# COMPiLELab/krylov_robustness

Measured on NVIDIA B200. Metric: krylov_matvecs_per_sec, higher is better.
Workload: dtype f64

## Files before the change

### krylov_robustness_b200/csrc/api.cu

```cuda
#include <memory>
#include <thread>
#include "common.cuh"
#include "csr.cuh"
#include "spmm.cuh"
#include "dense.cuh"
#include "slq.cuh"
#include "theta_table.h"
#include "smalldense.cuh"
#include "pairs.cuh"
#include "pairs_small.cuh"
#include "expmv.cuh"
#include "tsdense.cuh"
#include "smallgemm.cuh"
#include "vecops.cuh"
#include "blockkrylov.cuh"
#include "entries.cuh"
#include "entries_local.cuh"
#include "frechet.cuh"
#include "mctrace.cuh"
#include "nodepairs.cuh"

using namespace kr;

static void destroy_fun_update_result(kr_ctx* c);
// ... 295 lines not shown
        launch_spmm(ctx, A->dev, xb.p(), xb.panels, epi, nullptr, (int)k);
        download_cm(ctx, yb, Y, ldy);
    });
}

static void slq_finish(const SlqResult& R, int64_t m, double* tr, double* vals, double* alpha, double* beta) {
    if (tr) *tr = R.tr;
    const size_t k = R.vals.size();
    if (vals) std::memcpy(vals, R.vals.data(), k * sizeof(double));
    if (alpha || beta)
        for (int64_t j = 0; j < m; ++j)
            for (size_t c = 0; c < k; ++c) {
                if (alpha) alpha[c * m + j] = R.alpha[(size_t)j * k + c];
                if (beta) beta[c * m + j] = R.beta[(size_t)j * k + c];
            }
}

int kr_slq_trace_dev(kr_ctx* ctx, const kr_matrix* A, const kr_dense* Z, int64_t m, int fun, double* tr,
                     double* vals, double* alpha, double* beta) {
    return guarded([&] {
        if (!ctx || !A || !Z) fail(KR_ERR_ARG, "kr_slq_trace_dev: null argument");
        if (fun < 0 || fun > 2) fail(KR_ERR_ARG, "unsupported function selector");
        KR_CUDA(cudaSetDevice(ctx->device));
        PanelBuf W(ctx, Z->buf.n, Z->buf.cols);
        KR_CUDA(cudaMemcpyAsync(W.p(), Z->buf.p(), (size_t)W.elems() * sizeof(double), cudaMemcpyDeviceToDevice,
                                ctx->stream));
        SlqResult R = slq_run(ctx, A, W, (int)m, fun, alpha || beta);
        slq_finish(R, m, tr, vals, alpha, beta);
    });
}

}

template <class T>
static int slq_trace_host(kr_ctx* ctx, const kr_matrix* A, int64_t k, const T* Z, int64_t ldz, int64_t m, int fun,
                          double* tr, double* vals, double* alpha, double* beta) {
    return guarded([&] {
        if (!ctx || !A || !Z) fail(KR_ERR_ARG, "kr_slq_trace: null argument");
        if (fun < 0 || fun > 2) fail(KR_ERR_ARG, "unsupported function selector");
        KR_CUDA(cudaSetDevice(ctx->device));
        const int64_t n = A->dev.n;
        if (ldz < n) fail(KR_ERR_ARG, "The block vector b has wrong number of rows");
        if (k <= 0) fail(KR_ERR_ARG, "kr_slq_trace: no probe columns");
        std::vector<int64_t> cstart, cwidth;
        for (int64_t c0 = 0; c0 < k;) {
            const int64_t cw = std::min<int64_t>(k - c0, cstart.empty() ? 2 * PW : (cstart.size() == 1 ? 6 * PW : 8 * PW));
            cstart.push_back(c0);
            cwidth.push_back(cw);
            c0 += cw;
        }
        if (cstart.empty()) { cstart.push_back(0); cwidth.push_back(0); }
        const int64_t nch = (int64_t)cstart.size();
        if (!ctx->copy_stream) KR_CUDA(cudaStreamCreateWithFlags(&ctx->copy_stream, cudaStreamNonBlocking));
        std::vector<std::unique_ptr<PanelBuf>> W(nch);
        std::vector<std::unique_ptr<DevBuf<T>>> stage(nch);
        std::vector<cudaEvent_t> ready(nch, nullptr);
        for (int64_t c = 0; c < nch; ++c) {
            W[c].reset(new PanelBuf(ctx, n, (int)cwidth[c]));
            stage[c].reset(new DevBuf<T>(ctx, (size_t)std::max<int64_t>(n * cwidth[c], 1)));
        }
        KR_CUDA(cudaStreamSynchronize(ctx->stream));
        auto issue_copy = [&](int64_t c) {
            const int64_t c0 = cstart[c], cw = cwidth[c];
            if (n > 0 && cw > 0) {
                KR_CUDA(cudaMemcpy2DAsync(stage[c]->p, n * sizeof(T), Z + c0 * ldz, ldz * sizeof(T),
                                          n * sizeof(T), cw, cudaMemcpyHostToDevice, ctx->copy_stream));
                ctx->counters[3] += n * cw * (int64_t)sizeof(T);
            }
            cm_to_panel(ctx, stage[c]->p, n, *W[c], ctx->copy_stream);
            KR_CUDA(cudaEventCreateWithFlags(&ready[c], cudaEventDisableTiming));
            KR_CUDA(cudaEventRecord(ready[c], ctx->copy_stream));
        };
        std::vector<double> all_vals((size_t)k), all_a, all_b;
        if (alpha || beta) { all_a.resize((size_t)m * k); all_b.resize((size_t)m * k); }
        auto harvest = [&](int64_t c, SlqJob& job) {
            const int64_t c0 = cstart[c], cw = cwidth[c];
            SlqResult R = job.collect();
            for (int64_t q = 0; q < cw; ++q) all_vals[(size_t)(c0 + q)] = R.vals[(size_t)q];
            if (alpha || beta)
                for (int64_t j = 0; j < m; ++j)
                    for (int64_t q = 0; q < cw; ++q) {
                        all_a[(size_t)(j * k + c0 + q)] = R.alpha[(size_t)(j * cw + q)];
                        all_b[(size_t)(j * k + c0 + q)] = R.beta[(size_t)(j * cw + q)];
                    }
        };
        try {
            issue_copy(0);
            std::unique_ptr<SlqJob> prev;
            for (int64_t c = 0; c < nch; ++c) {
                KR_CUDA(cudaStreamWaitEvent(ctx->stream, ready[c], 0));
                std::unique_ptr<SlqJob> job(new SlqJob(ctx, A, *W[c], (int)m, fun, alpha || beta));
                job->mark();
                if (c + 1 < nch) issue_copy(c + 1);
                if (prev) harvest(c - 1, *prev);
                prev = std::move(job);
            }
            if (prev) harvest(nch - 1, *prev);
        } catch (...) {
            cudaStreamSynchronize(ctx->copy_stream);
            cudaStreamSynchronize(ctx->stream);
            for (auto e : ready) if (e) cudaEventDestroy(e);
            throw;
        }
        KR_CUDA(cudaStreamSynchronize(ctx->copy_stream));
        for (auto e : ready) if (e) cudaEventDestroy(e);
        SlqResult R;
        R.vals = all_vals;
        R.alpha = all_a;
        R.beta = all_b;
        double s = 0.0;
        for (int64_t q = 0; q < k; ++q) s += all_vals[(size_t)q];
        R.tr = k ? s / (double)k : 0.0;
        slq_finish(R, m, tr, vals, alpha, beta);
    });
// ... 53 lines not shown
```

### krylov_robustness_b200/csrc/csr.cuh

```cuda
#pragma once
#include <algorithm>
#include <map>
#include <numeric>

#include "common.cuh"

namespace kr {

struct RowTile {
    int start;
    int count;
    int lanes_log2;
    int pad;
};

struct CsrHost {
    int64_t n = 0;
    std::vector<int64_t> row_ptr;
    std::vector<int32_t> col;
    std::vector<double> val;
};

struct CsrDevView {
    int n;
// ... 12 lines not shown
    const double* __restrict__ dl_val;
    int dl_count;
};

#ifndef KR_SPMM_CAP
#define KR_SPMM_CAP 4096
#endif
#ifndef KR_SPMM_MAX_ROWS
#define KR_SPMM_MAX_ROWS 1024
#endif
constexpr int SPMM_CAP = KR_SPMM_CAP;
constexpr int SPMM_MAX_ROWS = KR_SPMM_MAX_ROWS;
constexpr int SPMM_LONG_ROW = 1024;
constexpr int64_t CSR_L2_RESIDENT_NNZ = 400000;

struct CsrDev {
    int64_t n = 0, nnz = 0;
    DevBuf<int> row_ptr, col, row_order, row_pos;
    DevBuf<double> val;
    DevBuf<RowTile> tiles;
    DevBuf<int> dl_tile_begin, dl_rowlocal, dl_pos, dl_col;
    DevBuf<double> dl_val;
    int dl_count = 0;
    std::vector<RowTile> tiles_host;
    std::vector<int> row_pos_host;
    int ntiles = 0;
    bool pattern_only = false;
    double uval = 1.0;
    CsrDevView view() const {
        CsrDevView v;
        v.n = (int)n;
        v.ntiles = ntiles;
        v.row_ptr = row_ptr.p;
        v.col = col.p;
        v.val = pattern_only ? nullptr : val.p;
        v.uval = uval;
        v.row_order = row_order.p;
        v.row_pos = row_pos.p;
        v.tiles = tiles.p;
        const bool dl = dl_count > 0;
        v.dl_tile_begin = dl ? dl_tile_begin.p : nullptr;
        v.dl_rowlocal = dl ? dl_rowlocal.p : nullptr;
        v.dl_pos = dl ? dl_pos.p : nullptr;
        v.dl_col = dl ? dl_col.p : nullptr;
        v.dl_val = dl ? dl_val.p : nullptr;
        v.dl_count = dl_count;
// ... 119 lines not shown
    D.nnz = nnz;
    D.pattern_only = P.uniform;
    D.uval = P.uval;
    D.row_ptr.reset(ctx, n + 1);
    D.row_ptr.upload(P.srp.data(), n + 1);
    D.col.reset(ctx, std::max<int64_t>(nnz, 1));
    if (nnz) D.col.upload(P.scol.data(), nnz);
    if (!P.uniform) {
        D.val.reset(ctx, std::max<int64_t>(nnz, 1));
        if (nnz) D.val.upload(P.sval.data(), nnz);
    } else {
        D.val.free();
    }
    D.ntiles = (int)P.tiles.size();
    D.row_order.reset(ctx, std::max<int64_t>(n, 1));
    if (n) D.row_order.upload(P.order.data(), n);
    std::vector<int> pos((size_t)std::max<int64_t>(n, 1), 0);
    for (int64_t s = 0; s < n; ++s) pos[(size_t)P.order[(size_t)s]] = (int)s;
    D.row_pos.reset(ctx, std::max<int64_t>(n, 1));
    if (n) D.row_pos.upload(pos.data(), n);
    D.tiles_host = P.tiles;
    D.row_pos_host = pos;
    D.dl_count = 0;
    D.tiles.reset(ctx, std::max<size_t>(P.tiles.size(), 1));
    if (!P.tiles.empty()) D.tiles.upload(P.tiles.data(), P.tiles.size());
    KR_CUDA(cudaStreamSynchronize(ctx->stream));
}

}

struct kr_matrix {
    kr_ctx* ctx = nullptr;
    kr::CsrHost host;
    std::map<std::pair<int64_t, int64_t>, double> pending;
    kr::CsrDev dev;
    kr::CsrDev devT;
    bool symmetric = true;
    bool nonnegative = true;
    double trace = 0.0;
    double norm1 = 0.0;
    std::vector<kr_matrix*> peers;
    bool is_peer = false;
    const kr::CsrDev& T() const { return symmetric ? dev : devT; }
};

namespace kr {
// ... 146 lines not shown
```

### krylov_robustness_b200/csrc/dense.cuh

```cuda
#pragma once
#include "spmm.cuh"

namespace kr {

struct PanelBuf {
    DevBuf<double> buf;
    int64_t n = 0;
    int cols = 0, panels = 0;
    PanelBuf() = default;
    PanelBuf(kr_ctx* ctx, int64_t n_, int cols_) { reset(ctx, n_, cols_); }
    void reset(kr_ctx* ctx, int64_t n_, int cols_) {
        n = n_;
        cols = cols_;
        panels = (cols_ + PW - 1) / PW;
        buf.reset(ctx, (size_t)n * panels * PW);
    }
    double* p() const { return buf.p; }
    int64_t elems() const { return n * panels * PW; }
};

__global__ void __launch_bounds__(256)
cm_to_panel_kernel(const double* __restrict__ src, int64_t ld, int64_t n, int cols,
                   double* __restrict__ dst) {
    __shared__ double t[PW][65];
    const int q = blockIdx.y;
    const int64_t r0 = (int64_t)blockIdx.x * 64;
    for (int e = threadIdx.x; e < PW * 64; e += 256) {
        int c = e / 64, i = e % 64;
        int64_t r = r0 + i;
        int col = q * PW + c;
        t[c][i] = (r < n && col < cols) ? src[r + (int64_t)col * ld] : 0.0;
    }
    __syncthreads();
    double* d = dst + (int64_t)q * n * PW + r0 * PW;
    for (int e = threadIdx.x; e < PW * 64; e += 256) {
        int i = e / PW, c = e % PW;
        if (r0 + i < n) d[e] = t[c][i];
    }
}

__global__ void __launch_bounds__(256)
panel_to_cm_kernel(const double* __restrict__ src, int64_t n, int cols, double* __restrict__ dst,
                   int64_t ld) {
    __shared__ double t[PW][65];
    const int q = blockIdx.y;
    const int64_t r0 = (int64_t)blockIdx.x * 64;
    const double* s = src + (int64_t)q * n * PW + r0 * PW;
    for (int e = threadIdx.x; e < PW * 64; e += 256) {
        int i = e / PW, c = e % PW;
        t[c][i] = (r0 + i < n) ? s[e] : 0.0;
    }
    __syncthreads();
    for (int e = threadIdx.x; e < PW * 64; e += 256) {
        int c = e / 64, i = e % 64;
        int64_t r = r0 + i;
        int col = q * PW + c;
        if (r < n && col < cols) dst[r + (int64_t)col * ld] = t[c][i];
    }
}

__global__ void __launch_bounds__(256)
cm_i8_to_panel_kernel(const signed char* __restrict__ src, int64_t ld, int64_t n, int cols,
                      double* __restrict__ dst) {
    __shared__ signed char t[PW][64 + 4];
    const int q = blockIdx.y;
    const int64_t r0 = (int64_t)blockIdx.x * 64;
    for (int e = threadIdx.x; e < PW * 64; e += 256) {
        int c = e / 64, i = e % 64;
        int64_t r = r0 + i;
        int col = q * PW + c;
        t[c][i] = (r < n && col < cols) ? src[r + (int64_t)col * ld] : (signed char)0;
    }
    __syncthreads();
    double* d = dst + (int64_t)q * n * PW + r0 * PW;
    for (int e = threadIdx.x; e < PW * 64; e += 256) {
        int i = e / PW, c = e % PW;
        const int v = t[c][i];
        if (r0 + i < n) d[e] = v > 0 ? 1.0 : (v < 0 ? -1.0 : 0.0);
    }
}
inline void cm_to_panel(kr_ctx* ctx, const signed char* src_dev, int64_t ld, PanelBuf& dst, cudaStream_t stream = nullptr) {
    if (dst.n == 0 || dst.panels == 0) return;
    dim3 grid((unsigned)ceil_div(dst.n, 64), (unsigned)dst.panels);
    cm_i8_to_panel_kernel<<<grid, 256, 0, stream ? stream : ctx->stream>>>(src_dev, ld, dst.n, dst.cols, dst.p());
    check_launch(ctx, "cm_i8_to_panel_kernel");
}
inline void cm_to_panel(kr_ctx* ctx, const double* src_dev, int64_t ld, PanelBuf& dst, cudaStream_t stream = nullptr) {
    if (dst.n == 0 || dst.panels == 0) return;
    dim3 grid((unsigned)ceil_div(dst.n, 64), (unsigned)dst.panels);
    cm_to_panel_kernel<<<grid, 256, 0, stream ? stream : ctx->stream>>>(src_dev, ld, dst.n, dst.cols, dst.p());
    check_launch(ctx, "cm_to_panel_kernel");
}
inline void panel_to_cm(kr_ctx* ctx, const PanelBuf& src, double* dst_dev, int64_t ld) {
    if (src.n == 0 || src.panels == 0) return;
    dim3 grid((unsigned)ceil_div(src.n, 64), (unsigned)src.panels);
    KR_LAUNCH(ctx, panel_to_cm_kernel, grid, 256, 0, src.p(), src.n, src.cols, dst_dev, ld);
}

__host__ __device__ inline uint64_t splitmix64(uint64_t x) {
    x += 0x9E3779B97F4A7C15ull;
    x = (x ^ (x >> 30)) * 0xBF58476D1CE4E5B9ull;
    x = (x ^ (x >> 27)) * 0x94D049BB133111EBull;
    return x ^ (x >> 31);
}
__global__ void rademacher_kernel(double* __restrict__ dst, int64_t n, int cols, int panels,
                                  uint64_t seed, int64_t col_offset) {
    const int64_t total = n * panels * PW;
    for (int64_t e = (int64_t)blockIdx.x * blockDim.x + threadIdx.x; e < total;
         e += (int64_t)gridDim.x * blockDim.x) {
        int64_t q = e / (n * PW), rem = e % (n * PW);
        int64_t i = rem / PW;
        int c = (int)(q * PW + rem % PW);
        double v = 0.0;
        if (c < cols) {
// ... 15 lines not shown
}

__global__ void __launch_bounds__(COL_THREADS)
colnorm2_kernel(const double* __restrict__ X, int64_t n, double* __restrict__ partial, int total_cols) {
    __shared__ double smem[COL_WARPS * LPT * 2];
    const int q = blockIdx.y, sub = threadIdx.x % LPT;
    const double* Xp = X + (int64_t)q * n * PW;
    const int64_t r0 = (int64_t)blockIdx.x * COL_ROWS_PER_CTA;
    const int64_t r1 = min(n, r0 + COL_ROWS_PER_CTA);
    double acc[2] = {0.0, 0.0};
    for (int64_t r = r0 + (threadIdx.x / LPT); r < r1; r += COL_THREADS / LPT) {
        double2 x = *reinterpret_cast<const double2*>(Xp + r * PW + sub * 2);
        acc[0] += x.x * x.x;
        acc[1] += x.y * x.y;
    }
    col_cta_reduce<2>(acc, smem);
    if (threadIdx.x < LPT) {
        double* o = partial + (int64_t)blockIdx.x * total_cols + q * PW + threadIdx.x * 2;
        o[0] = acc[0];
        o[1] = acc[1];
    }
}

__global__ void __launch_bounds__(COL_THREADS)
combine3_norm_kernel(const double* __restrict__ Y, const double* __restrict__ U1,
                     const double* U0, double* W, int64_t n, const double* __restrict__ coef,
                     int total_cols, double* __restrict__ partial) {
    __shared__ double smem[COL_WARPS * LPT * 2];
    const int q = blockIdx.y, sub = threadIdx.x % LPT;
    const int64_t po = (int64_t)q * n * PW;
    const int col = q * PW + sub * 2;
    const double c0x = coef[col], c0y = coef[col + 1];
    const double c1x = coef[total_cols + col], c1y = coef[total_cols + col + 1];
    const double c2x = coef[2 * total_cols + col], c2y = coef[2 * total_cols + col + 1];
    const int64_t r0 = (int64_t)blockIdx.x * COL_ROWS_PER_CTA;
    const int64_t r1 = min(n, r0 + COL_ROWS_PER_CTA);
    double acc[2] = {0.0, 0.0};
    for (int64_t r = r0 + (threadIdx.x / LPT); r < r1; r += COL_THREADS / LPT) {
        const int64_t o = po + r * PW + sub * 2;
        double2 y = __ldcs(reinterpret_cast<const double2*>(Y + o));
        double2 u1 = *reinterpret_cast<const double2*>(U1 + o);
        double2 u0 = *reinterpret_cast<const double2*>(U0 + o);
        double2 w;
        w.x = c0x * y.x + c1x * u1.x + c2x * u0.x;
        w.y = c0y * y.y + c1y * u1.y + c2y * u0.y;
        *reinterpret_cast<double2*>(W + o) = w;
        acc[0] += w.x * w.x;
        acc[1] += w.y * w.y;
    }
    col_cta_reduce<2>(acc, smem);
    if (threadIdx.x < LPT) {
        double* o = partial + (int64_t)blockIdx.x * total_cols + q * PW + threadIdx.x * 2;
        o[0] = acc[0];
        o[1] = acc[1];
    }
}

__global__ void __launch_bounds__(256)
sum_partials_kernel(const double* __restrict__ partial, int nblocks, int total_cols,
                    double* __restrict__ out) {
    __shared__ double sm[8][33];
    const int tx = threadIdx.x & 31, ty = threadIdx.x >> 5;
    const int c = blockIdx.x * 32 + tx;
    double s = 0.0;
    if (c < total_cols)
        for (int b = ty; b < nblocks; b += 8) s += partial[(int64_t)b * total_cols + c];
    sm[ty][tx] = s;
    __syncthreads();
// ... 46 lines not shown
    int c = blockIdx.x * blockDim.x + threadIdx.x;
    if (c >= total_cols) return;
    const double d = sums[c];
    nrm2[c] = d;
    st.s1[c] = d > 0.0 ? 1.0 / sqrt(d) : 0.0;
    st.s0[c] = 0.0;
    st.beta_prev[c] = 0.0;
}

__device__ __forceinline__ double apply_fun(int fun, double x) {
    return fun == KR_FUN_EXP ? exp(x) : fun == KR_FUN_SINH ? sinh(x) : cosh(x);
}

constexpr int SLQ_MAX_M = 128;
__global__ void slq_quadrature_kernel(const double* __restrict__ alpha, const double* __restrict__ beta,
                                      const double* __restrict__ nrm2, int m, int cols, int total_cols,
                                      int fun, double* __restrict__ vals) {
    int c = blockIdx.x * blockDim.x + threadIdx.x;
    if (c >= cols) return;
    double d[SLQ_MAX_M], e[SLQ_MAX_M], z[SLQ_MAX_M];
    int n = m;
    for (int i = 0; i < m; ++i) {
        d[i] = alpha[(int64_t)i * total_cols + c];
        e[i] = beta[(int64_t)i * total_cols + c];
        z[i] = 0.0;
        if (n == m && !(e[i] > 0.0)) n = i + 1;
    }
    e[n - 1] = 0.0;
    z[0] = 1.0;
    for (int l = 0; l < n; ++l) {
        int iter = 0, mm;
        do {
            for (mm = l; mm < n - 1; ++mm) {
                double dd = fabs(d[mm]) + fabs(d[mm + 1]);
                if (fabs(e[mm]) <= 2.220446049250313e-16 * dd) break;
            }
            if (mm != l) {
                if (iter++ == 100) break;
                double g = (d[l + 1] - d[l]) / (2.0 * e[l]);
                double r = hypot(g, 1.0);
                g = d[mm] - d[l] + e[l] / (g + copysign(r, g));
                double s = 1.0, cc = 1.0, p = 0.0;
                int i;
                for (i = mm - 1; i >= l; --i) {
                    double f = s * e[i], b = cc * e[i];
                    r = hypot(f, g);
                    e[i + 1] = r;
                    if (r == 0.0) {
                        d[i + 1] -= p;
// ... 28 lines not shown
```

### krylov_robustness_b200/csrc/slq.cuh

```cuda
#pragma once
#include "dense.cuh"

namespace kr {

struct SlqResult {
    double tr = 0.0;
    std::vector<double> vals, alpha, beta;
};

struct SlqJob {
    kr_ctx* ctx;
    int m, cols, tc;
    bool want_ab;
    PanelBuf B2, Y;
    DevBuf<double> partial, sums, scal, alpha, beta, vals;

    SlqJob(kr_ctx* c, const kr_matrix* M, PanelBuf& Z, int m_, int fun, bool want_ab_) : ctx(c), m(m_), want_ab(want_ab_) {
        if (m < 1 || m > SLQ_MAX_M) fail(KR_ERR_ARG, "slq: m must be in 1..%d", SLQ_MAX_M);
        const CsrDev& A = M->dev;
        const int64_t n = A.n;
        if (Z.n != n) fail(KR_ERR_ARG, "The block vector b has wrong number of rows");
        cols = Z.cols;
        const int panels = Z.panels;
        tc = panels * PW;
        B2.reset(ctx, n, cols);
        Y.reset(ctx, n, cols);
        B2.buf.zero();
        const int rb = col_row_blocks(n);
        const int nparts = std::max(rb, A.ntiles);
        partial.reset(ctx, (size_t)nparts * tc);
        sums.reset(ctx, tc);
        scal.reset(ctx, (size_t)tc * 7);
        alpha.reset(ctx, (size_t)m * tc);
        beta.reset(ctx, (size_t)m * tc);
        vals.reset(ctx, tc);
        scal.zero();
        SlqState st;
        st.s1 = scal.p;
        st.s0 = scal.p + tc;
        st.beta_prev = scal.p + 2 * tc;
        st.coef = scal.p + 3 * tc;
        double* nrm2 = scal.p + 6 * tc;
        st.alpha = alpha.p;
        st.beta = beta.p;
        const int sb = (int)ceil_div(tc, 128);
        dim3 cgrid((unsigned)rb, (unsigned)panels);
        KR_LAUNCH(ctx, colnorm2_kernel, cgrid, COL_THREADS, 0, Z.p(), n, partial.p, tc);
        sum_partials(ctx, partial.p, rb, tc, sums.p);
        KR_LAUNCH(ctx, slq_init_kernel, sb, 128, 0, sums.p, tc, st, nrm2);
        double* U1 = Z.p();
        double* U0 = B2.p();
        for (int j = 0; j < m; ++j) {
            EpiDot epi;
            epi.Y = Y.p();
            epi.X = U1;
            epi.partial = partial.p;
            epi.total_cols = tc;
            launch_spmm(ctx, A, U1, panels, epi, nullptr, cols);
            sum_partials(ctx, partial.p, A.ntiles, tc, sums.p);
            KR_LAUNCH(ctx, slq_alpha_kernel, sb, 128, 0, sums.p, tc, st, j);
            KR_LAUNCH(ctx, combine3_norm_kernel, cgrid, COL_THREADS, 0, Y.p(), U1, U0, U0, n, st.coef, tc, partial.p);
            sum_partials(ctx, partial.p, rb, tc, sums.p);
            KR_LAUNCH(ctx, slq_beta_kernel, sb, 128, 0, sums.p, tc, st, j);
            std::swap(U0, U1);
        }
        KR_LAUNCH(ctx, slq_quadrature_kernel, (int)ceil_div(cols, 64), 64, 0, alpha.p, beta.p, nrm2, m, cols, tc, fun, vals.p);
    }

    cudaEvent_t finished = nullptr;
    void mark() {
        KR_CUDA(cudaEventCreateWithFlags(&finished, cudaEventDisableTiming));
        KR_CUDA(cudaEventRecord(finished, ctx->stream));
    }
    ~SlqJob() { if (finished) cudaEventDestroy(finished); }

    SlqResult collect() {
        SlqResult R;
        std::vector<double> v(vals.count);
        if (finished) {
            KR_CUDA(cudaEventSynchronize(finished));
            cudaStream_t cs = ctx->copy_stream ? ctx->copy_stream : ctx->stream;
            KR_CUDA(cudaMemcpyAsync(v.data(), vals.p, v.size() * sizeof(double), cudaMemcpyDeviceToHost, cs));
            KR_CUDA(cudaStreamSynchronize(cs));
            ctx->counters[4] += (int64_t)(v.size() * sizeof(double));
        } else {
            v = vals.to_host();
        }
        R.vals.assign(v.begin(), v.begin() + cols);
        double s = 0.0;
        for (int c = 0; c < cols; ++c) s += R.vals[c];
        R.tr = cols ? s / cols : 0.0;
        if (want_ab) {
            if (finished) KR_CUDA(cudaStreamSynchronize(ctx->stream));
            std::vector<double> a = alpha.to_host(), b = beta.to_host();
            R.alpha.resize((size_t)m * cols);
            R.beta.resize((size_t)m * cols);
            for (int j = 0; j < m; ++j)
                for (int c = 0; c < cols; ++c) {
                    R.alpha[(size_t)j * cols + c] = a[(size_t)j * tc + c];
                    R.beta[(size_t)j * cols + c] = b[(size_t)j * tc + c];
                }
        }
        return R;
    }
};

inline SlqResult slq_run(kr_ctx* ctx, const kr_matrix* M, PanelBuf& Z, int m, int fun, bool want_ab) {
    SlqJob job(ctx, M, Z, m, fun, want_ab);
    return job.collect();
}

}
```

### krylov_robustness_b200/csrc/spmm.cuh

```cuda
#pragma once
#include "csr.cuh"

namespace kr {

#ifndef KR_PW
#define KR_PW 16
#endif
constexpr int PW = KR_PW;
constexpr int LPT = PW / 2;
static_assert(PW == 8 || PW == 16, "panel width must be 8 or 16");
#ifndef KR_SPMM_THREADS
#define KR_SPMM_THREADS 256
#endif
constexpr int SPMM_THREADS = KR_SPMM_THREADS;
constexpr int COL_WARPS = 8;
constexpr int SPMM_WARPS = SPMM_THREADS / 32;
#ifndef KR_SPMM_MIN_CTAS
#define KR_SPMM_MIN_CTAS 4
#endif
constexpr int SPMM_MIN_CTAS = KR_SPMM_MIN_CTAS;

struct PanelBlock {
    double* p;
    int64_t n;
// ... 87 lines not shown
    double* __restrict__ Y;
    const double* __restrict__ X;
    double alpha, mu;
    __device__ __forceinline__ void init(int q, int64_t stride) {
        Y += q * stride;
        X += q * stride;
    }
    Vec<CPL> xr;
    __device__ __forceinline__ void pre(int r, int sub) {
        if (mu != 0.0 && sub == 0) prefetch_l1(X + (int64_t)r * PW);
    }
    __device__ __forceinline__ void row(int r, int sub, Vec<CPL> y, unsigned) {
        if (mu != 0.0) xr = ld_row(X + (int64_t)r * PW + sub * CPL);
#pragma unroll
        for (int i = 0; i < CPL; ++i) {
            if (mu != 0.0) y.v[i] -= mu * xr.v[i];
            y.v[i] *= alpha;
        }
        st_stream(Y + (int64_t)r * PW + sub * CPL, y);
    }
    __device__ __forceinline__ void finish(int, int, double*) {}
};

struct EpiDot {
    static constexpr int CPL = 4;
    double* __restrict__ Y;
    const double* __restrict__ X;
    double* __restrict__ partial;
    int total_cols;
    double acc[CPL];
    __device__ __forceinline__ void init(int q, int64_t stride) {
        Y += q * stride;
        X += q * stride;
#pragma unroll
        for (int i = 0; i < CPL; ++i) acc[i] = 0.0;
    }
    Vec<CPL> xr;
    __device__ __forceinline__ void pre(int r, int sub) {
        if (sub == 0) prefetch_l1(X + (int64_t)r * PW);
    }
    __device__ __forceinline__ void row(int r, int sub, Vec<CPL> y, unsigned) {
        xr = ld_row(X + (int64_t)r * PW + sub * CPL);
#pragma unroll
        for (int i = 0; i < CPL; ++i) acc[i] += xr.v[i] * y.v[i];
        st_stream(Y + (int64_t)r * PW + sub * CPL, y);
    }
    __device__ __forceinline__ void finish(int tile, int panel, double* smem) {
        cta_reduce_by_sub<CPL, SPMM_WARPS, PW / CPL>(acc, smem);
        if (threadIdx.x < PW / CPL) {
            double* o = partial + (int64_t)tile * total_cols + panel * PW + threadIdx.x * CPL;
#pragma unroll
            for (int i = 0; i < CPL; ++i) o[i] = acc[i];
        }
    }
};

struct EpiGram2 {
    static constexpr int CPL = 2;
    double* __restrict__ Y;
    const double* __restrict__ P;
    const double* __restrict__ C;
    double* __restrict__ partial;
    int ncand;
    double acc[8];
    __device__ __forceinline__ void init(int q, int64_t stride) {
        Y += q * stride;
        C += q * stride;
        if (P) P += q * stride;
// ... 176 lines not shown
template <bool HAS_VAL, int U, int CPL>
__device__ __forceinline__ Vec<CPL> gather_accumulate(int p_first, int p_end, int stride, const int* __restrict__ scol,
                                                      const double* __restrict__ sval, const double* __restrict__ xs,
                                                      const double* __restrict__ xpanel, int pf_sub) {
    Vec<CPL> acc0 = vzero<CPL>(), acc1 = vzero<CPL>();
    int p = p_first;
    for (; p + (U - 1) * stride < p_end; p += U * stride) {
#if KR_SPMM_PF > 0
        if (CPL == 2) {
            const int qpf = p + (KR_SPMM_PF * U + pf_sub) * stride;
            if (pf_sub < U && qpf < p_end) prefetch_x(xpanel + (int64_t)scol[qpf] * PW);
        }
#endif
        gather_block<HAS_VAL, U, CPL, false>(p, p_end, stride, scol, sval, xs, acc0, acc1);
    }
    if (p < p_end) gather_block<HAS_VAL, U, CPL, true>(p, p_end, stride, scol, sval, xs, acc0, acc1);
    if (CPL == 2) {
#pragma unroll
        for (int i = 0; i < CPL; ++i) acc0.v[i] += acc1.v[i];
    }
    return acc0;
}

template <int L, bool HAS_VAL, int U, bool DELTA, class Epi>
__device__ __forceinline__ void spmm_tile(const RowTile t, const int* __restrict__ srp, const int* __restrict__ srid,
                                          const int* __restrict__ scol, const double* __restrict__ sval,
                                          const double* __restrict__ Xp, double uval, Epi& epi, const CsrDevView& A,
                                          int e0, int e1) {
    constexpr int CPL = Epi::CPL;
    constexpr int LP = PW / CPL;
    constexpr int S = L / LP;
    constexpr int RPW = 32 / L;
    const int lane = threadIdx.x & 31, warp = threadIdx.x >> 5;
    const int sub = lane % LP;
    const int slot = (lane % L) / LP;
    const int rlocal = lane / L;
    const double* xs = Xp + sub * CPL;
    for (int base = warp * RPW; base < t.count; base += SPMM_WARPS * RPW) {
        const int rr = base + rlocal;
        const bool valid = rr < t.count;
        int row = 0, p0 = 0, p1 = 0;
        if (valid) {
            row = srid[rr];
            p0 = srp[rr];
            p1 = srp[rr + 1];
        }
        const bool emit = valid && slot == 0;
        if (emit) epi.pre(row, sub);
#if KR_SPMM_PF > 0
        if (CPL == 2) {
            const int rn = rr + KR_SPMM_PF * SPMM_WARPS * RPW;
            if (rn < t.count) {
                const int q0 = srp[rn], q1 = srp[rn + 1];
#pragma unroll
                for (int k = 0; k < KR_SPMM_PF; ++k) {
                    const int q = q0 + slot + (k * U + sub) * S;
                    if (sub < U && q < q1) prefetch_x(Xp + (int64_t)scol[q] * PW);
                }
            }
        }
#endif
        Vec<CPL> acc = gather_accumulate<HAS_VAL, U, CPL>(p0 + slot, p1, S, scol, sval, xs, Xp, sub);
#pragma unroll
        for (int off = LP; off < L; off <<= 1) {
#pragma unroll
            for (int i = 0; i < CPL; ++i) acc.v[i] += __shfl_xor_sync(0xffffffffu, acc.v[i], off);
        }
        if (!HAS_VAL) {
#pragma unroll
            for (int i = 0; i < CPL; ++i) acc.v[i] *= uval;
        }
        if (DELTA && e1 > e0 && emit) {
            for (int e = e0; e < e1; ++e)
                if (A.dl_rowlocal[e] == rr) {
                    const Vec<CPL> x = ld_x<CPL>(xs + (int64_t)A.dl_col[e] * PW);
                    const double d = A.dl_val[e];
#pragma unroll
                    for (int i = 0; i < CPL; ++i) acc.v[i] = fma(d, x.v[i], acc.v[i]);
                }
        }
        const unsigned m = __ballot_sync(0xffffffffu, emit);
        if (emit) epi.row(row, sub, acc, m);
    }
}

template <class Epi, bool HAS_VAL, int U, bool DELTA>
__device__ __forceinline__ void spmm_item(const CsrDevView& A, const double* __restrict__ X, const Epi& epi_proto,
                                          int64_t panel_stride, int tile, int panel, double* red, unsigned char* dyn_smem) {
    constexpr int CPL = Epi::CPL;
    constexpr int LP = PW / CPL;
    int* scol = reinterpret_cast<int*>(dyn_smem);
    int* srp = scol + SPMM_CAP;
    int* srid = srp + SPMM_MAX_ROWS + 1;
    double* sval = reinterpret_cast<double*>(dyn_smem + SPMM_SMEM_PATTERN);
    const RowTile t = A.tiles[tile];
    const int pb = __ldg(A.row_ptr + t.start);
    const int nz = __ldg(A.row_ptr + t.start + t.count) - pb;
    const bool long_row = t.lanes_log2 == 6;
    const int e0 = DELTA && A.dl_tile_begin ? A.dl_tile_begin[tile] : 0;
    const int e1 = DELTA && A.dl_tile_begin ? A.dl_tile_begin[tile + 1] : 0;
    Epi epi = epi_proto;
    epi.init(panel, panel_stride);
    const double* Xp = X + (int64_t)panel * panel_stride;
    if (!long_row) {
        for (int i = threadIdx.x; i <= t.count; i += SPMM_THREADS) srp[i] = __ldg(A.row_ptr + t.start + i) - pb;
        for (int i = threadIdx.x; i < t.count; i += SPMM_THREADS) srid[i] = __ldg(A.row_order + t.start + i);
        for (int p = threadIdx.x; p < nz; p += SPMM_THREADS) scol[p] = ld_stream(A.col + pb + p);
        if (HAS_VAL)
            for (int p = threadIdx.x; p < nz; p += SPMM_THREADS) sval[p] = ld_stream(A.val + pb + p);
        __syncthreads();
        switch (t.lanes_log2) {
            case 0: spmm_tile<LP, HAS_VAL, U, DELTA>(t, srp, srid, scol, sval, Xp, A.uval, epi, A, e0, e1); break;
            case 1: spmm_tile<2 * LP, HAS_VAL, U, DELTA>(t, srp, srid, scol, sval, Xp, A.uval, epi, A, e0, e1); break;
            case 2: spmm_tile<(4 * LP > 32 ? 32 : 4 * LP), HAS_VAL, U, DELTA>(t, srp, srid, scol, sval, Xp, A.uval, epi, A, e0, e1); break;
            default: spmm_tile<(8 * LP > 32 ? 32 : 8 * LP), HAS_VAL, U, DELTA>(t, srp, srid, scol, sval, Xp, A.uval, epi, A, e0, e1); break;
        }
    } else {
        const int sub = threadIdx.x % LP, slot = threadIdx.x / LP;
        const int row = __ldg(A.row_order + t.start);
        const bool emit = threadIdx.x < LP;
        if (emit) epi.pre(row, sub);
        double v[CPL];
#pragma unroll
        for (int i = 0; i < CPL; ++i) v[i] = 0.0;
        for (int c0 = 0; c0 < nz; c0 += SPMM_CAP) {
            const int cn = min(SPMM_CAP, nz - c0);
            __syncthreads();
            for (int p = threadIdx.x; p < cn; p += SPMM_THREADS) scol[p] = ld_stream(A.col + pb + c0 + p);
            if (HAS_VAL)
                for (int p = threadIdx.x; p < cn; p += SPMM_THREADS) sval[p] = ld_stream(A.val + pb + c0 + p);
            __syncthreads();
            Vec<CPL> a = gather_accumulate<HAS_VAL, U, CPL>(slot, cn, SPMM_THREADS / LP, scol, sval, Xp + sub * CPL, Xp, sub);
#pragma unroll
            for (int i = 0; i < CPL; ++i) v[i] += a.v[i];
        }
        cta_reduce_by_sub<CPL, SPMM_WARPS, LP>(v, red);
        Vec<CPL> acc;
#pragma unroll
        for (int i = 0; i < CPL; ++i) acc.v[i] = HAS_VAL ? v[i] : v[i] * A.uval;
        if (DELTA && e1 > e0 && emit) {
            for (int e = e0; e < e1; ++e) {
                const Vec<CPL> x = ld_x<CPL>(Xp + sub * CPL + (int64_t)A.dl_col[e] * PW);
                const double d = A.dl_val[e];
#pragma unroll
                for (int i = 0; i < CPL; ++i) acc.v[i] = fma(d, x.v[i], acc.v[i]);
            }
        }
        const unsigned m = __ballot_sync(0xffffffffu, emit);
        if (emit) epi.row(row, sub, acc, m);
        __syncthreads();
    }
    epi.finish(tile, panel, red);
}

template <class Epi, bool HAS_VAL, int U, bool DELTA>
__global__ void __launch_bounds__(SPMM_THREADS, SPMM_MIN_CTAS)
spmm_kernel(CsrDevView A, const double* __restrict__ X, Epi epi_proto, int64_t panel_stride,
            const int* __restrict__ done, const int* __restrict__ panel_active) {
    if (done && *done) return;
    const int panel = blockIdx.y;
    if (panel_active && !panel_active[panel]) return;
    __shared__ double red[SPMM_WARPS * LPT * 8];
    extern __shared__ __align__(16) unsigned char dyn_smem[];
    spmm_item<Epi, HAS_VAL, U, DELTA>(A, X, epi_proto, panel_stride, (int)blockIdx.x, panel, red, dyn_smem);
}


inline bool first_use_on_device(bool (&flags)[64], int device) {
    if (device < 0 || device >= 64 || flags[device]) return false;
    flags[device] = true;
    return true;
}

template <class Epi, int U>
inline void launch_spmm_impl(kr_ctx* ctx, const CsrDev& A, const double* X, int panels, const Epi& epi,
                             const int* done, const int* panel_active) {
    static bool attr_set[64] = {};
    if (first_use_on_device(attr_set, ctx->device)) {
        KR_CUDA(cudaFuncSetAttribute(spmm_kernel<Epi, false, U, false>, cudaFuncAttributeMaxDynamicSharedMemorySize, (int)SPMM_SMEM_PATTERN));
        KR_CUDA(cudaFuncSetAttribute(spmm_kernel<Epi, true, U, false>, cudaFuncAttributeMaxDynamicSharedMemorySize, (int)SPMM_SMEM_VALUED));
        KR_CUDA(cudaFuncSetAttribute(spmm_kernel<Epi, false, U, true>, cudaFuncAttributeMaxDynamicSharedMemorySize, (int)SPMM_SMEM_PATTERN));
        KR_CUDA(cudaFuncSetAttribute(spmm_kernel<Epi, true, U, true>, cudaFuncAttributeMaxDynamicSharedMemorySize, (int)SPMM_SMEM_VALUED));
    }
    const int64_t ps = (int64_t)A.n * PW;
    const dim3 grid((unsigned)A.ntiles, (unsigned)panels);
    if (A.dl_count > 0) {
        if (A.pattern_only) spmm_kernel<Epi, false, U, true><<<grid, SPMM_THREADS, SPMM_SMEM_PATTERN, ctx->stream>>>(A.view(), X, epi, ps, done, panel_active);
        else spmm_kernel<Epi, true, U, true><<<grid, SPMM_THREADS, SPMM_SMEM_VALUED, ctx->stream>>>(A.view(), X, epi, ps, done, panel_active);
    } else {
        if (A.pattern_only) spmm_kernel<Epi, false, U, false><<<grid, SPMM_THREADS, SPMM_SMEM_PATTERN, ctx->stream>>>(A.view(), X, epi, ps, done, panel_active);
        else spmm_kernel<Epi, true, U, false><<<grid, SPMM_THREADS, SPMM_SMEM_VALUED, ctx->stream>>>(A.view(), X, epi, ps, done, panel_active);
    }
}

#ifndef KR_SPMM_U2
#define KR_SPMM_U2 8
#endif
#ifndef KR_SPMM_U4
#define KR_SPMM_U4 4
#endif

template <class Epi>
inline void launch_spmm(kr_ctx* ctx, const CsrDev& A, const double* X, int panels, const Epi& epi,
                        const int* done = nullptr, int logical_cols = -1, const int* panel_active = nullptr) {
    if (A.ntiles == 0 || panels == 0) return;
    cudaEvent_t e0 = nullptr, e1 = nullptr;
    if (ctx->timing) {
        ctx->timing_events(&e0, &e1);
        KR_CUDA(cudaEventRecord(e0, ctx->stream));
    }
    launch_spmm_impl<Epi, Epi::CPL == 4 ? KR_SPMM_U4 : KR_SPMM_U2>(ctx, A, X, panels, epi, done, panel_active);
    check_launch(ctx, "spmm_kernel");
    if (ctx->timing) {
        KR_CUDA(cudaEventRecord(e1, ctx->stream));
        ctx->spmm_events.emplace_back(e0, e1);
    }
    ctx->counters[1] += 1;
    ctx->counters[2] += logical_cols >= 0 ? logical_cols : (int64_t)panels * PW;
}

}
```

Baseline: 49340.

## Run SLQ Lanczos in stored row order and trim first/last iteration work

Permutes the probe vectors into the matrix's tiled row order once, when they are loaded. It builds a cached column array remapped through row_pos, so the SpMM kernel can skip the row_order indirection and write Y contiguously in stored order. It also drops the zero-fill of the second basis buffer by specialising the first combine step without a U0 term, and skips storing Y on the final alpha-only SpMM. This costs an extra nnz-sized column array, scattered writes in the panel conversion, and a permuted gather for device-side inputs.

```diff
diff --git a/krylov_robustness_b200/csrc/api.cu b/krylov_robustness_b200/csrc/api.cu
--- a/krylov_robustness_b200/csrc/api.cu
+++ b/krylov_robustness_b200/csrc/api.cu
@@ -341,10 +341,13 @@
         if (!ctx || !A || !Z) fail(KR_ERR_ARG, "kr_slq_trace_dev: null argument");
         if (fun < 0 || fun > 2) fail(KR_ERR_ARG, "unsupported function selector");
         KR_CUDA(cudaSetDevice(ctx->device));
+        if (Z->buf.n != A->dev.n) fail(KR_ERR_ARG, "The block vector b has wrong number of rows");
         PanelBuf W(ctx, Z->buf.n, Z->buf.cols);
-        KR_CUDA(cudaMemcpyAsync(W.p(), Z->buf.p(), (size_t)W.elems() * sizeof(double), cudaMemcpyDeviceToDevice,
-                                ctx->stream));
-        SlqResult R = slq_run(ctx, A, W, (int)m, fun, alpha || beta);
+        const bool stored = slq_prepare_stored_order(ctx, A);
+        if (stored) rows_to_stored(ctx, Z->buf, A->dev.row_order.p, W);
+        else KR_CUDA(cudaMemcpyAsync(W.p(), Z->buf.p(), (size_t)W.elems() * sizeof(double), cudaMemcpyDeviceToDevice,
+                                     ctx->stream));
+        SlqResult R = slq_run(ctx, A, W, (int)m, fun, alpha || beta, stored);
         slq_finish(R, m, tr, vals, alpha, beta);
     });
 }
@@ -378,6 +381,8 @@
             W[c].reset(new PanelBuf(ctx, n, (int)cwidth[c]));
             stage[c].reset(new DevBuf<T>(ctx, (size_t)std::max<int64_t>(n * cwidth[c], 1)));
         }
+        const bool stored = slq_prepare_stored_order(ctx, A);
+        const int* row_pos = stored ? A->dev.row_pos.p : nullptr;
         KR_CUDA(cudaStreamSynchronize(ctx->stream));
         auto issue_copy = [&](int64_t c) {
             const int64_t c0 = cstart[c], cw = cwidth[c];
@@ -386,7 +391,7 @@
                                           n * sizeof(T), cw, cudaMemcpyHostToDevice, ctx->copy_stream));
                 ctx->counters[3] += n * cw * (int64_t)sizeof(T);
             }
-            cm_to_panel(ctx, stage[c]->p, n, *W[c], ctx->copy_stream);
+            cm_to_panel(ctx, stage[c]->p, n, *W[c], ctx->copy_stream, row_pos);
             KR_CUDA(cudaEventCreateWithFlags(&ready[c], cudaEventDisableTiming));
             KR_CUDA(cudaEventRecord(ready[c], ctx->copy_stream));
         };
@@ -408,7 +413,7 @@
             std::unique_ptr<SlqJob> prev;
             for (int64_t c = 0; c < nch; ++c) {
                 KR_CUDA(cudaStreamWaitEvent(ctx->stream, ready[c], 0));
-                std::unique_ptr<SlqJob> job(new SlqJob(ctx, A, *W[c], (int)m, fun, alpha || beta));
+                std::unique_ptr<SlqJob> job(new SlqJob(ctx, A, *W[c], (int)m, fun, alpha || beta, stored));
                 job->mark();
                 if (c + 1 < nch) issue_copy(c + 1);
                 if (prev) harvest(c - 1, *prev);
diff --git a/krylov_robustness_b200/csrc/csr.cuh b/krylov_robustness_b200/csrc/csr.cuh
--- a/krylov_robustness_b200/csrc/csr.cuh
+++ b/krylov_robustness_b200/csrc/csr.cuh
@@ -58,6 +58,8 @@
     DevBuf<int> dl_tile_begin, dl_rowlocal, dl_pos, dl_col;
     DevBuf<double> dl_val;
     int dl_count = 0;
+    DevBuf<int> col_stored;
+    bool col_stored_ready = false;
     std::vector<RowTile> tiles_host;
     std::vector<int> row_pos_host;
     int ntiles = 0;
@@ -223,6 +225,8 @@
     D.tiles_host = P.tiles;
     D.row_pos_host = pos;
     D.dl_count = 0;
+    D.col_stored.free();
+    D.col_stored_ready = false;
     D.tiles.reset(ctx, std::max<size_t>(P.tiles.size(), 1));
     if (!P.tiles.empty()) D.tiles.upload(P.tiles.data(), P.tiles.size());
     KR_CUDA(cudaStreamSynchronize(ctx->stream));
diff --git a/krylov_robustness_b200/csrc/dense.cuh b/krylov_robustness_b200/csrc/dense.cuh
--- a/krylov_robustness_b200/csrc/dense.cuh
+++ b/krylov_robustness_b200/csrc/dense.cuh
@@ -21,7 +21,7 @@
 
 __global__ void __launch_bounds__(256)
 cm_to_panel_kernel(const double* __restrict__ src, int64_t ld, int64_t n, int cols,
-                   double* __restrict__ dst) {
+                   double* __restrict__ dst, const int* __restrict__ row_pos) {
     __shared__ double t[PW][65];
     const int q = blockIdx.y;
     const int64_t r0 = (int64_t)blockIdx.x * 64;
@@ -32,10 +32,11 @@
         t[c][i] = (r < n && col < cols) ? src[r + (int64_t)col * ld] : 0.0;
     }
     __syncthreads();
-    double* d = dst + (int64_t)q * n * PW + r0 * PW;
+    double* d = dst + (int64_t)q * n * PW;
     for (int e = threadIdx.x; e < PW * 64; e += 256) {
         int i = e / PW, c = e % PW;
-        if (r0 + i < n) d[e] = t[c][i];
+        const int64_t r = r0 + i;
+        if (r < n) d[(row_pos ? (int64_t)row_pos[r] : r) * PW + c] = t[c][i];
     }
 }
 
@@ -61,7 +62,7 @@
 
 __global__ void __launch_bounds__(256)
 cm_i8_to_panel_kernel(const signed char* __restrict__ src, int64_t ld, int64_t n, int cols,
-                      double* __restrict__ dst) {
+                      double* __restrict__ dst, const int* __restrict__ row_pos) {
     __shared__ signed char t[PW][64 + 4];
     const int q = blockIdx.y;
     const int64_t r0 = (int64_t)blockIdx.x * 64;
@@ -72,24 +73,43 @@
         t[c][i] = (r < n && col < cols) ? src[r + (int64_t)col * ld] : (signed char)0;
     }
     __syncthreads();
-    double* d = dst + (int64_t)q * n * PW + r0 * PW;
+    double* d = dst + (int64_t)q * n * PW;
     for (int e = threadIdx.x; e < PW * 64; e += 256) {
         int i = e / PW, c = e % PW;
         const int v = t[c][i];
-        if (r0 + i < n) d[e] = v > 0 ? 1.0 : (v < 0 ? -1.0 : 0.0);
-    }
-}
-inline void cm_to_panel(kr_ctx* ctx, const signed char* src_dev, int64_t ld, PanelBuf& dst, cudaStream_t stream = nullptr) {
+        const int64_t r = r0 + i;
+        if (r < n) d[(row_pos ? (int64_t)row_pos[r] : r) * PW + c] = v > 0 ? 1.0 : (v < 0 ? -1.0 : 0.0);
+    }
+}
+inline void cm_to_panel(kr_ctx* ctx, const signed char* src_dev, int64_t ld, PanelBuf& dst, cudaStream_t stream = nullptr,
+                        const int* row_pos = nullptr) {
     if (dst.n == 0 || dst.panels == 0) return;
     dim3 grid((unsigned)ceil_div(dst.n, 64), (unsigned)dst.panels);
-    cm_i8_to_panel_kernel<<<grid, 256, 0, stream ? stream : ctx->stream>>>(src_dev, ld, dst.n, dst.cols, dst.p());
+    cm_i8_to_panel_kernel<<<grid, 256, 0, stream ? stream : ctx->stream>>>(src_dev, ld, dst.n, dst.cols, dst.p(), row_pos);
     check_launch(ctx, "cm_i8_to_panel_kernel");
 }
-inline void cm_to_panel(kr_ctx* ctx, const double* src_dev, int64_t ld, PanelBuf& dst, cudaStream_t stream = nullptr) {
+inline void cm_to_panel(kr_ctx* ctx, const double* src_dev, int64_t ld, PanelBuf& dst, cudaStream_t stream = nullptr,
+                        const int* row_pos = nullptr) {
     if (dst.n == 0 || dst.panels == 0) return;
     dim3 grid((unsigned)ceil_div(dst.n, 64), (unsigned)dst.panels);
-    cm_to_panel_kernel<<<grid, 256, 0, stream ? stream : ctx->stream>>>(src_dev, ld, dst.n, dst.cols, dst.p());
+    cm_to_panel_kernel<<<grid, 256, 0, stream ? stream : ctx->stream>>>(src_dev, ld, dst.n, dst.cols, dst.p(), row_pos);
     check_launch(ctx, "cm_to_panel_kernel");
+}
+
+__global__ void __launch_bounds__(256)
+rows_to_stored_kernel(const double* __restrict__ src, const int* __restrict__ row_order, int64_t n, int64_t tiles,
+                      double* __restrict__ dst) {
+    for (int64_t e = (int64_t)blockIdx.x * blockDim.x + threadIdx.x; e < tiles * LPT; e += (int64_t)gridDim.x * blockDim.x) {
+        const int64_t t = e / LPT, q = t / n, s = t % n;
+        const int sub = (int)(e % LPT);
+        const double2 v = __ldcs(reinterpret_cast<const double2*>(src + (q * n + row_order[s]) * PW) + sub);
+        __stcs(reinterpret_cast<double2*>(dst + t * PW) + sub, v);
+    }
+}
+inline void rows_to_stored(kr_ctx* ctx, const PanelBuf& src, const int* row_order, PanelBuf& dst) {
+    const int64_t tiles = src.n * src.panels;
+    if (tiles == 0) return;
+    KR_LAUNCH(ctx, rows_to_stored_kernel, ctx->num_sms * 16, 256, 0, src.p(), row_order, src.n, tiles, dst.p());
 }
 inline void panel_to_cm(kr_ctx* ctx, const PanelBuf& src, double* dst_dev, int64_t ld) {
     if (src.n == 0 || src.panels == 0) return;
@@ -151,6 +171,7 @@
     }
 }
 
+template <bool HAS_U0>
 __global__ void __launch_bounds__(COL_THREADS)
 combine3_norm_kernel(const double* __restrict__ Y, const double* __restrict__ U1,
                      const double* U0, double* W, int64_t n, const double* __restrict__ coef,
@@ -169,10 +190,14 @@
         const int64_t o = po + r * PW + sub * 2;
         double2 y = __ldcs(reinterpret_cast<const double2*>(Y + o));
         double2 u1 = *reinterpret_cast<const double2*>(U1 + o);
-        double2 u0 = *reinterpret_cast<const double2*>(U0 + o);
         double2 w;
-        w.x = c0x * y.x + c1x * u1.x + c2x * u0.x;
-        w.y = c0y * y.y + c1y * u1.y + c2y * u0.y;
+        w.x = c0x * y.x + c1x * u1.x;
+        w.y = c0y * y.y + c1y * u1.y;
+        if (HAS_U0) {
+            double2 u0 = *reinterpret_cast<const double2*>(U0 + o);
+            w.x += c2x * u0.x;
+            w.y += c2y * u0.y;
+        }
         *reinterpret_cast<double2*>(W + o) = w;
         acc[0] += w.x * w.x;
         acc[1] += w.y * w.y;
@@ -265,9 +290,9 @@
     int n = m;
     for (int i = 0; i < m; ++i) {
         d[i] = alpha[(int64_t)i * total_cols + c];
-        e[i] = beta[(int64_t)i * total_cols + c];
+        e[i] = i < m - 1 ? beta[(int64_t)i * total_cols + c] : 0.0;
         z[i] = 0.0;
-        if (n == m && !(e[i] > 0.0)) n = i + 1;
+        if (n == m && i < m - 1 && !(e[i] > 0.0)) n = i + 1;
     }
     e[n - 1] = 0.0;
     z[0] = 1.0;
diff --git a/krylov_robustness_b200/csrc/slq.cuh b/krylov_robustness_b200/csrc/slq.cuh
--- a/krylov_robustness_b200/csrc/slq.cuh
+++ b/krylov_robustness_b200/csrc/slq.cuh
@@ -8,14 +8,21 @@
     std::vector<double> vals, alpha, beta;
 };
 
+inline bool slq_prepare_stored_order(kr_ctx* ctx, const kr_matrix* M) {
+    if (!M->symmetric || M->dev.dl_count > 0) return false;
+    prepare_stored_cols(ctx, const_cast<kr_matrix*>(M)->dev);
+    return true;
+}
+
 struct SlqJob {
     kr_ctx* ctx;
     int m, cols, tc;
-    bool want_ab;
+    bool want_ab, stored;
     PanelBuf B2, Y;
     DevBuf<double> partial, sums, scal, alpha, beta, vals;
 
-    SlqJob(kr_ctx* c, const kr_matrix* M, PanelBuf& Z, int m_, int fun, bool want_ab_) : ctx(c), m(m_), want_ab(want_ab_) {
+    SlqJob(kr_ctx* c, const kr_matrix* M, PanelBuf& Z, int m_, int fun, bool want_ab_, bool stored_)
+        : ctx(c), m(m_), want_ab(want_ab_), stored(stored_) {
         if (m < 1 || m > SLQ_MAX_M) fail(KR_ERR_ARG, "slq: m must be in 1..%d", SLQ_MAX_M);
         const CsrDev& A = M->dev;
         const int64_t n = A.n;
@@ -25,7 +32,6 @@
         tc = panels * PW;
         B2.reset(ctx, n, cols);
         Y.reset(ctx, n, cols);
-        B2.buf.zero();
         const int rb = col_row_blocks(n);
         const int nparts = std::max(rb, A.ntiles);
         partial.reset(ctx, (size_t)nparts * tc);
@@ -49,22 +55,34 @@
         sum_partials(ctx, partial.p, rb, tc, sums.p);
         KR_LAUNCH(ctx, slq_init_kernel, sb, 128, 0, sums.p, tc, st, nrm2);
         double* U1 = Z.p();
-        double* U0 = B2.p();
+        double* U0 = nullptr;
         for (int j = 0; j < m; ++j) {
-            EpiDot epi;
-            epi.Y = Y.p();
-            epi.X = U1;
-            epi.partial = partial.p;
-            epi.total_cols = tc;
-            launch_spmm(ctx, A, U1, panels, epi, nullptr, cols);
+            const bool last_alpha_only = j == m - 1 && !want_ab;
+            if (last_alpha_only) spmm_dot<false>(A, U1, panels);
+            else spmm_dot<true>(A, U1, panels);
             sum_partials(ctx, partial.p, A.ntiles, tc, sums.p);
             KR_LAUNCH(ctx, slq_alpha_kernel, sb, 128, 0, sums.p, tc, st, j);
-            KR_LAUNCH(ctx, combine3_norm_kernel, cgrid, COL_THREADS, 0, Y.p(), U1, U0, U0, n, st.coef, tc, partial.p);
+            if (last_alpha_only) break;
+            double* W = U0 ? U0 : B2.p();
+            if (U0) KR_LAUNCH(ctx, combine3_norm_kernel<true>, cgrid, COL_THREADS, 0, Y.p(), U1, U0, W, n, st.coef, tc, partial.p);
+            else KR_LAUNCH(ctx, combine3_norm_kernel<false>, cgrid, COL_THREADS, 0, Y.p(), U1, nullptr, W, n, st.coef, tc, partial.p);
             sum_partials(ctx, partial.p, rb, tc, sums.p);
             KR_LAUNCH(ctx, slq_beta_kernel, sb, 128, 0, sums.p, tc, st, j);
-            std::swap(U0, U1);
+            U0 = U1;
+            U1 = W;
         }
         KR_LAUNCH(ctx, slq_quadrature_kernel, (int)ceil_div(cols, 64), 64, 0, alpha.p, beta.p, nrm2, m, cols, tc, fun, vals.p);
+    }
+
+    template <bool STORE_Y>
+    void spmm_dot(const CsrDev& A, const double* U, int panels) {
+        EpiDotT<STORE_Y> epi;
+        epi.Y = Y.p();
+        epi.X = U;
+        epi.partial = partial.p;
+        epi.total_cols = tc;
+        if (stored) launch_spmm<EpiDotT<STORE_Y>, true>(ctx, A, U, panels, epi, nullptr, cols);
+        else launch_spmm(ctx, A, U, panels, epi, nullptr, cols);
     }
 
     cudaEvent_t finished = nullptr;
@@ -105,8 +123,8 @@
     }
 };
 
-inline SlqResult slq_run(kr_ctx* ctx, const kr_matrix* M, PanelBuf& Z, int m, int fun, bool want_ab) {
-    SlqJob job(ctx, M, Z, m, fun, want_ab);
+inline SlqResult slq_run(kr_ctx* ctx, const kr_matrix* M, PanelBuf& Z, int m, int fun, bool want_ab, bool stored) {
+    SlqJob job(ctx, M, Z, m, fun, want_ab, stored);
     return job.collect();
 }
 
diff --git a/krylov_robustness_b200/csrc/spmm.cuh b/krylov_robustness_b200/csrc/spmm.cuh
--- a/krylov_robustness_b200/csrc/spmm.cuh
+++ b/krylov_robustness_b200/csrc/spmm.cuh
@@ -133,7 +133,8 @@
     __device__ __forceinline__ void finish(int, int, double*) {}
 };
 
-struct EpiDot {
+template <bool STORE_Y>
+struct EpiDotT {
     static constexpr int CPL = 4;
     double* __restrict__ Y;
     const double* __restrict__ X;
@@ -154,7 +155,7 @@
         xr = ld_row(X + (int64_t)r * PW + sub * CPL);
 #pragma unroll
         for (int i = 0; i < CPL; ++i) acc[i] += xr.v[i] * y.v[i];
-        st_stream(Y + (int64_t)r * PW + sub * CPL, y);
+        if (STORE_Y) st_stream(Y + (int64_t)r * PW + sub * CPL, y);
     }
     __device__ __forceinline__ void finish(int tile, int panel, double* smem) {
         cta_reduce_by_sub<CPL, SPMM_WARPS, PW / CPL>(acc, smem);
@@ -377,7 +378,7 @@
     return acc0;
 }
 
-template <int L, bool HAS_VAL, int U, bool DELTA, class Epi>
+template <int L, bool HAS_VAL, int U, bool DELTA, bool STORED, class Epi>
 __device__ __forceinline__ void spmm_tile(const RowTile t, const int* __restrict__ srp, const int* __restrict__ srid,
                                           const int* __restrict__ scol, const double* __restrict__ sval,
                                           const double* __restrict__ Xp, double uval, Epi& epi, const CsrDevView& A,
@@ -396,7 +397,7 @@
         const bool valid = rr < t.count;
         int row = 0, p0 = 0, p1 = 0;
         if (valid) {
-            row = srid[rr];
+            row = STORED ? t.start + rr : srid[rr];
             p0 = srp[rr];
             p1 = srp[rr + 1];
         }
@@ -439,7 +440,7 @@
     }
 }
 
-template <class Epi, bool HAS_VAL, int U, bool DELTA>
+template <class Epi, bool HAS_VAL, int U, bool DELTA, bool STORED>
 __device__ __forceinline__ void spmm_item(const CsrDevView& A, const double* __restrict__ X, const Epi& epi_proto,
                                           int64_t panel_stride, int tile, int panel, double* red, unsigned char* dyn_smem) {
     constexpr int CPL = Epi::CPL;
@@ -459,20 +460,21 @@
     const double* Xp = X + (int64_t)panel * panel_stride;
     if (!long_row) {
         for (int i = threadIdx.x; i <= t.count; i += SPMM_THREADS) srp[i] = __ldg(A.row_ptr + t.start + i) - pb;
-        for (int i = threadIdx.x; i < t.count; i += SPMM_THREADS) srid[i] = __ldg(A.row_order + t.start + i);
+        if (!STORED)
+            for (int i = threadIdx.x; i < t.count; i += SPMM_THREADS) srid[i] = __ldg(A.row_order + t.start + i);
         for (int p = threadIdx.x; p < nz; p += SPMM_THREADS) scol[p] = ld_stream(A.col + pb + p);
         if (HAS_VAL)
             for (int p = threadIdx.x; p < nz; p += SPMM_THREADS) sval[p] = ld_stream(A.val + pb + p);
         __syncthreads();
         switch (t.lanes_log2) {
-            case 0: spmm_tile<LP, HAS_VAL, U, DELTA>(t, srp, srid, scol, sval, Xp, A.uval, epi, A, e0, e1); break;
-            case 1: spmm_tile<2 * LP, HAS_VAL, U, DELTA>(t, srp, srid, scol, sval, Xp, A.uval, epi, A, e0, e1); break;
-            case 2: spmm_tile<(4 * LP > 32 ? 32 : 4 * LP), HAS_VAL, U, DELTA>(t, srp, srid, scol, sval, Xp, A.uval, epi, A, e0, e1); break;
-            default: spmm_tile<(8 * LP > 32 ? 32 : 8 * LP), HAS_VAL, U, DELTA>(t, srp, srid, scol, sval, Xp, A.uval, epi, A, e0, e1); break;
+            case 0: spmm_tile<LP, HAS_VAL, U, DELTA, STORED>(t, srp, srid, scol, sval, Xp, A.uval, epi, A, e0, e1); break;
+            case 1: spmm_tile<2 * LP, HAS_VAL, U, DELTA, STORED>(t, srp, srid, scol, sval, Xp, A.uval, epi, A, e0, e1); break;
+            case 2: spmm_tile<(4 * LP > 32 ? 32 : 4 * LP), HAS_VAL, U, DELTA, STORED>(t, srp, srid, scol, sval, Xp, A.uval, epi, A, e0, e1); break;
+            default: spmm_tile<(8 * LP > 32 ? 32 : 8 * LP), HAS_VAL, U, DELTA, STORED>(t, srp, srid, scol, sval, Xp, A.uval, epi, A, e0, e1); break;
         }
     } else {
         const int sub = threadIdx.x % LP, slot = threadIdx.x / LP;
-        const int row = __ldg(A.row_order + t.start);
+        const int row = STORED ? t.start : __ldg(A.row_order + t.start);
         const bool emit = threadIdx.x < LP;
         if (emit) epi.pre(row, sub);
         double v[CPL];
@@ -508,7 +510,7 @@
     epi.finish(tile, panel, red);
 }
 
-template <class Epi, bool HAS_VAL, int U, bool DELTA>
+template <class Epi, bool HAS_VAL, int U, bool DELTA, bool STORED>
 __global__ void __launch_bounds__(SPMM_THREADS, SPMM_MIN_CTAS)
 spmm_kernel(CsrDevView A, const double* __restrict__ X, Epi epi_proto, int64_t panel_stride,
             const int* __restrict__ done, const int* __restrict__ panel_active) {
@@ -517,7 +519,7 @@
     if (panel_active && !panel_active[panel]) return;
     __shared__ double red[SPMM_WARPS * LPT * 8];
     extern __shared__ __align__(16) unsigned char dyn_smem[];
-    spmm_item<Epi, HAS_VAL, U, DELTA>(A, X, epi_proto, panel_stride, (int)blockIdx.x, panel, red, dyn_smem);
+    spmm_item<Epi, HAS_VAL, U, DELTA, STORED>(A, X, epi_proto, panel_stride, (int)blockIdx.x, panel, red, dyn_smem);
 }
 
 
@@ -527,24 +529,50 @@
     return true;
 }
 
-template <class Epi, int U>
+__global__ void stored_cols_kernel(const int* __restrict__ col, const int* __restrict__ row_pos, int64_t nnz,
+                                   int* __restrict__ out) {
+    for (int64_t p = (int64_t)blockIdx.x * blockDim.x + threadIdx.x; p < nnz; p += (int64_t)gridDim.x * blockDim.x)
+        out[p] = row_pos[col[p]];
+}
+inline void prepare_stored_cols(kr_ctx* ctx, CsrDev& A) {
+    if (A.col_stored_ready) return;
+    A.col_stored.reset(ctx, (size_t)std::max<int64_t>(A.nnz, 1));
+    if (A.nnz > 0) KR_LAUNCH(ctx, stored_cols_kernel, ctx->num_sms * 8, 256, 0, A.col.p, A.row_pos.p, A.nnz, A.col_stored.p);
+    A.col_stored_ready = true;
+}
+
+template <class Epi, int U, bool STORED>
 inline void launch_spmm_impl(kr_ctx* ctx, const CsrDev& A, const double* X, int panels, const Epi& epi,
                              const int* done, const int* panel_active) {
     static bool attr_set[64] = {};
-    if (first_use_on_device(attr_set, ctx->device)) {
-        KR_CUDA(cudaFuncSetAttribute(spmm_kernel<Epi, false, U, false>, cudaFuncAttributeMaxDynamicSharedMemorySize, (int)SPMM_SMEM_PATTERN));
-        KR_CUDA(cudaFuncSetAttribute(spmm_kernel<Epi, true, U, false>, cudaFuncAttributeMaxDynamicSharedMemorySize, (int)SPMM_SMEM_VALUED));
-        KR_CUDA(cudaFuncSetAttribute(spmm_kernel<Epi, false, U, true>, cudaFuncAttributeMaxDynamicSharedMemorySize, (int)SPMM_SMEM_PATTERN));
-        KR_CUDA(cudaFuncSetAttribute(spmm_kernel<Epi, true, U, true>, cudaFuncAttributeMaxDynamicSharedMemorySize, (int)SPMM_SMEM_VALUED));
-    }
     const int64_t ps = (int64_t)A.n * PW;
     const dim3 grid((unsigned)A.ntiles, (unsigned)panels);
-    if (A.dl_count > 0) {
-        if (A.pattern_only) spmm_kernel<Epi, false, U, true><<<grid, SPMM_THREADS, SPMM_SMEM_PATTERN, ctx->stream>>>(A.view(), X, epi, ps, done, panel_active);
-        else spmm_kernel<Epi, true, U, true><<<grid, SPMM_THREADS, SPMM_SMEM_VALUED, ctx->stream>>>(A.view(), X, epi, ps, done, panel_active);
+    if constexpr (STORED) {
+        if (!A.col_stored_ready || A.dl_count > 0) fail(KR_ERR_ARG, "spmm: stored-order view of A not prepared");
+        if (first_use_on_device(attr_set, ctx->device)) {
+            KR_CUDA(cudaFuncSetAttribute(spmm_kernel<Epi, false, U, false, true>, cudaFuncAttributeMaxDynamicSharedMemorySize, (int)SPMM_SMEM_PATTERN));
+            KR_CUDA(cudaFuncSetAttribute(spmm_kernel<Epi, true, U, false, true>, cudaFuncAttributeMaxDynamicSharedMemorySize, (int)SPMM_SMEM_VALUED));
+        }
+        CsrDevView v = A.view();
+        v.col = A.col_stored.p;
+        v.row_order = nullptr;
+        if (A.pattern_only) spmm_kernel<Epi, false, U, false, true><<<grid, SPMM_THREADS, SPMM_SMEM_PATTERN, ctx->stream>>>(v, X, epi, ps, done, panel_active);
+        else spmm_kernel<Epi, true, U, false, true><<<grid, SPMM_THREADS, SPMM_SMEM_VALUED, ctx->stream>>>(v, X, epi, ps, done, panel_active);
+        return;
     } else {
-        if (A.pattern_only) spmm_kernel<Epi, false, U, false><<<grid, SPMM_THREADS, SPMM_SMEM_PATTERN, ctx->stream>>>(A.view(), X, epi, ps, done, panel_active);
-        else spmm_kernel<Epi, true, U, false><<<grid, SPMM_THREADS, SPMM_SMEM_VALUED, ctx->stream>>>(A.view(), X, epi, ps, done, panel_active);
+        if (first_use_on_device(attr_set, ctx->device)) {
+            KR_CUDA(cudaFuncSetAttribute(spmm_kernel<Epi, false, U, false, false>, cudaFuncAttributeMaxDynamicSharedMemorySize, (int)SPMM_SMEM_PATTERN));
+            KR_CUDA(cudaFuncSetAttribute(spmm_kernel<Epi, true, U, false, false>, cudaFuncAttributeMaxDynamicSharedMemorySize, (int)SPMM_SMEM_VALUED));
+            KR_CUDA(cudaFuncSetAttribute(spmm_kernel<Epi, false, U, true, false>, cudaFuncAttributeMaxDynamicSharedMemorySize, (int)SPMM_SMEM_PATTERN));
+            KR_CUDA(cudaFuncSetAttribute(spmm_kernel<Epi, true, U, true, false>, cudaFuncAttributeMaxDynamicSharedMemorySize, (int)SPMM_SMEM_VALUED));
+        }
+        if (A.dl_count > 0) {
+            if (A.pattern_only) spmm_kernel<Epi, false, U, true, false><<<grid, SPMM_THREADS, SPMM_SMEM_PATTERN, ctx->stream>>>(A.view(), X, epi, ps, done, panel_active);
+            else spmm_kernel<Epi, true, U, true, false><<<grid, SPMM_THREADS, SPMM_SMEM_VALUED, ctx->stream>>>(A.view(), X, epi, ps, done, panel_active);
+        } else {
+            if (A.pattern_only) spmm_kernel<Epi, false, U, false, false><<<grid, SPMM_THREADS, SPMM_SMEM_PATTERN, ctx->stream>>>(A.view(), X, epi, ps, done, panel_active);
+            else spmm_kernel<Epi, true, U, false, false><<<grid, SPMM_THREADS, SPMM_SMEM_VALUED, ctx->stream>>>(A.view(), X, epi, ps, done, panel_active);
+        }
     }
 }
 
@@ -555,7 +583,7 @@
 #define KR_SPMM_U4 4
 #endif
 
-template <class Epi>
+template <class Epi, bool STORED = false>
 inline void launch_spmm(kr_ctx* ctx, const CsrDev& A, const double* X, int panels, const Epi& epi,
                         const int* done = nullptr, int logical_cols = -1, const int* panel_active = nullptr) {
     if (A.ntiles == 0 || panels == 0) return;
@@ -564,7 +592,7 @@
         ctx->timing_events(&e0, &e1);
         KR_CUDA(cudaEventRecord(e0, ctx->stream));
     }
-    launch_spmm_impl<Epi, Epi::CPL == 4 ? KR_SPMM_U4 : KR_SPMM_U2>(ctx, A, X, panels, epi, done, panel_active);
+    launch_spmm_impl<Epi, Epi::CPL == 4 ? KR_SPMM_U4 : KR_SPMM_U2, STORED>(ctx, A, X, panels, epi, done, panel_active);
     check_launch(ctx, "spmm_kernel");
     if (ctx->timing) {
         KR_CUDA(cudaEventRecord(e1, ctx->stream));
```

New measurement: 50280 (median of 6 runs). +1.9%, better.
